# samuel-vitorino/sopro

Hardware: AMD Instinct MI355X
Metric: audio_seconds_per_second (higher is better)
Workload: dtype f32; 1 GPU; Sopro-135M synthesize, 32 utterances x 200 frames per GPU (BASELINE configs[1]), S=64 text tokens, 32 distinct 150-frame reference voice(s) per batch prepared outside the timed region, top_p=0.9 T=1.05 anti_loop (reference defaults), synthetic weights with EOS suppressed; batch_per_gpu=32, frames=200, voices_per_batch=32, parallelism=replicas x1 (utterance sharding, no collective), lanes_per_gpu=4

## Files before the change

sopro_amd/csrc/seanet_uptail.hip:

```cpp
#include <type_traits>
#include <utility>

#include "common.h"

namespace {

constexpr int FC = 128;
constexpr int FTI = 32;
constexpr int FTS = 4 * FTI;
constexpr int FXR = FTI + 1;
constexpr int FXROW = 2 * FC * 2 + 16;
constexpr int FHROW = 272;
constexpr int FHLD = FHROW / 4;
constexpr int FHR = FTS + 2;
constexpr int FYROW = 144;
constexpr int FW1B = 2 * 6 * 2;
constexpr int FW2B = 2 * 2 * 2;
constexpr int FCARRY = 2 * FHROW;
constexpr int FXBUF = FXR * FXROW;
constexpr int FUSE_LDS = 2 * FXBUF + 2 * FHR * FHROW + FTS * FYROW + (FW1B + FW2B) * 1024 + 2 * FCARRY;
static_assert(FUSE_LDS <= 160 * 1024, "LDS");
static_assert(FXBUF % 16 == 0 && (FHR * FHROW) % 16 == 0 && (FTS * FYROW) % 16 == 0, "16-byte aligned LDS regions");

typedef __bf16 fbf16x8 __attribute__((ext_vector_type(8)));
typedef float ff32x4 __attribute__((ext_vector_type(4)));
__device__ __forceinline__ fbf16x8 ffrag(const uint4& v) { return *reinterpret_cast<const fbf16x8*>(&v); }

__device__ __forceinline__ void fsplit8(const float* __restrict__ p, uint4& hi, uint4& lo) {
  const float4 a = *reinterpret_cast<const float4*>(p), b = *reinterpret_cast<const float4*>(p + 4);
  split2_bf16(a.x, a.y, hi.x, lo.x);
  split2_bf16(a.z, a.w, hi.y, lo.y);
  split2_bf16(b.x, b.y, hi.z, lo.z);
  split2_bf16(b.z, b.w, hi.w, lo.w);
}

__device__ __forceinline__ unsigned pair_rows(unsigned mine, unsigned sel) {
  const unsigned got = (unsigned)__builtin_amdgcn_update_dpp(0, (int)mine, 0xB1 , 0xF, 0xF, true);
  return __builtin_amdgcn_perm(got, mine, sel);
}

template <int... I, class F>
__device__ __forceinline__ void sfor_impl(std::integer_sequence<int, I...>, F&& f) {
  (f(std::integral_constant<int, I>()), ...);
}
template <int N, class F>
__device__ __forceinline__ void sfor(F&& f) {
  sfor_impl(std::make_integer_sequence<int, N>(), f);
}
template <int V>
using IC = std::integral_constant<int, V>;

template <int PASSES, bool XH>
__global__ __launch_bounds__(512, 1) void seanet_uptail_kernel(const void* __restrict__ x_, int64_t x_seg_stride, const float* __restrict__ wu,
                                                               const float* __restrict__ bu, const float* __restrict__ w1,
                                                               const float* __restrict__ b1, const float* __restrict__ w2,
                                                               const float* __restrict__ b2, const float* __restrict__ wf, float bf,
                                                               float* __restrict__ wav, int64_t wav_seg_stride, int T, int tiles) {
  static_assert(PASSES == 1 || PASSES == 3, "passes");
  static_assert(!XH || PASSES == 1, "bf16 rows are a one-pass (bf16 mode) input form");
  extern __shared__ __attribute__((aligned(16))) unsigned char lds[];
  unsigned char* xs = lds;
  unsigned char* hs = xs + 2 * FXBUF;
  unsigned char* hp = hs + FHR * FHROW;
  unsigned char* ys = hp + FHR * FHROW;
  uint4* w1s = reinterpret_cast<uint4*>(ys + FTS * FYROW);
  uint4* w2s = w1s + FW1B * 64;
  uint4* chs = w2s + FW2B * 64;
  uint4* cps = chs + FCARRY / 16;

  const int tid = threadIdx.x, lane = tid & 63, wave = tid >> 6;
  const int b = blockIdx.y;
  const int frow = lane & 31, fg = lane >> 5;
  const int col = lane & 15, kq = lane >> 4;
  const int ph = wave >> 1, cbase = 32 * (wave & 1);
  const bool odd = (lane & 1) != 0;
  const unsigned pair_sel = odd ? 0x03020706u : 0x05040100u;
  const int ntile = (T + FTI - 1) / FTI;
  const int tile0 = (int)blockIdx.x * tiles;
  if (tile0 >= ntile) return;
  const int kfirst = tile0 > 0 ? tile0 - 1 : 0;
  const int klast = min(tile0 + tiles, ntile) - 1;
  const int S = 4 * T;
  const float* xb = XH ? nullptr : reinterpret_cast<const float*>(x_) + (int64_t)b * x_seg_stride;
  const unsigned short* xb16 = XH ? reinterpret_cast<const unsigned short*>(x_) + (int64_t)b * x_seg_stride : nullptr;
  float* wb = wav + (int64_t)b * wav_seg_stride;

  constexpr int NV = XH ? 2 : 3;
  auto request = [&](int t0, int q) -> uint4 {
    const int idx = tid + q * 512;
    const int rr = XH ? idx >> 4 : idx >> 5, cc = XH ? idx & 15 : idx & 31;
    const int p = t0 + rr;
    const int pc = (rr < FXR && p <= T) ? p : 0;
    if constexpr (XH) return bulk_load16(xb16 + (int64_t)pc * FC + cc * 8, true);
    else return bulk_load16(xb + (int64_t)pc * FC + cc * 4, true);
  };
  auto stage = [&](unsigned char* xbuf, int q, const uint4& val) {
    const int idx = tid + q * 512;
    const int rr = XH ? idx >> 4 : idx >> 5, cc = XH ? idx & 15 : idx & 31;
    if (rr < FXR) {
      if constexpr (XH) {
        *reinterpret_cast<uint4*>(xbuf + rr * FXROW + cc * 16) = val;
      } else {
        uint2 hi, lo;
        split2_bf16(__uint_as_float(val.x), __uint_as_float(val.y), hi.x, lo.x);
        split2_bf16(__uint_as_float(val.z), __uint_as_float(val.w), hi.y, lo.y);
        *reinterpret_cast<uint2*>(xbuf + rr * FXROW + cc * 8) = hi;
        if (PASSES == 3) *reinterpret_cast<uint2*>(xbuf + rr * FXROW + 2 * FC + cc * 8) = lo;
      }
    }
  };
  {
    uint4 v0[NV], v1[NV];
#pragma unroll
    for (int q = 0; q < NV; ++q) v0[q] = request(kfirst * FTI, q);
#pragma unroll
    for (int q = 0; q < NV; ++q) v1[q] = request((kfirst + 1) * FTI, q);
#pragma unroll
    for (int q = 0; q < NV; ++q) stage(xs + (kfirst & 1) * FXBUF, q, v0[q]);
#pragma unroll
    for (int q = 0; q < NV; ++q) stage(xs + ((kfirst + 1) & 1) * FXBUF, q, v1[q]);
  }

  uint4 wh[16], wl[PASSES == 3 ? 16 : 1];
#pragma unroll
  for (int s = 0; s < 16; ++s) {
    uint4 lo;
    fsplit8(wu + (int64_t)(wave * 32 + frow) * (2 * FC) + s * 16 + fg * 8, wh[s], lo);
    if (PASSES == 3) wl[s] = lo;
    if ((s & 3) == 3) asm volatile("" ::: "memory");
  }
  const float bv = bu[wave * 32 + frow];
  for (int c = wave; c < 12; c += 8) {
    const int nt = c / 6, s = c % 6;
    uint4 hi, lo;
    fsplit8(w1 + (16 * nt + col) * 192 + s * 32 + kq * 8, hi, lo);
    w1s[((nt * 6 + s) * 2 + 0) * 64 + lane] = hi;
    w1s[((nt * 6 + s) * 2 + 1) * 64 + lane] = lo;
  }
  if (wave < 4) {
    const int half = wave >> 1, s = wave & 1;
    uint4 hi, lo;
    fsplit8(w2 + (half * 32 + frow) * 32 + s * 16 + fg * 8, hi, lo);
    w2s[((half * 2 + s) * 2 + 0) * 64 + lane] = hi;
    w2s[((half * 2 + s) * 2 + 1) * 64 + lane] = lo;
  }
  uint4 w1r[PASSES == 1 ? 2 : 1][PASSES == 1 ? 6 : 1];
  if (PASSES == 1) {
#pragma unroll
    for (int nt = 0; nt < 2; ++nt)
#pragma unroll
      for (int s = 0; s < 6; ++s) {
        uint4 lo;
        fsplit8(w1 + (16 * nt + col) * 192 + s * 32 + kq * 8, w1r[PASSES == 1 ? nt : 0][PASSES == 1 ? s : 0], lo);
      }
  }
  if (tid < 2 * FCARRY / 16) chs[tid] = make_uint4(0u, 0u, 0u, 0u);
  const float b1v[2] = {b1[col], b1[16 + col]};
  const float b2v = b2[cbase + frow];
  const float wl0 = wf[lane], wl1 = wf[64 + lane], wl2 = wf[128 + lane];

  f32x16 accP;
  float hraw[16];
#pragma unroll
  for (int q = 0; q < 16; ++q) accP[q] = 0.f;

  constexpr int NP = 16 * PASSES;
  uint4 pah, pal, nah, nal;
  pal = nal = make_uint4(0u, 0u, 0u, 0u);
  auto p_read = [&](const unsigned char* xt, int s) {
    const unsigned char* p = xt + frow * FXROW + fg * 16 + (s >> 3) * FXROW + (s & 7) * 32;
    nah = *reinterpret_cast<const uint4*>(p);
    if (PASSES == 3) nal = *reinterpret_cast<const uint4*>(p + 2 * FC);
  };
  auto p_mfma = [&](const unsigned char* xt, auto j_) {
    constexpr int J = decltype(j_)::value, s = J / PASSES, piece = J % PASSES;
    if constexpr (piece == 0) {
      pah = nah;
      if (PASSES == 3) pal = nal;
      if constexpr (s + 1 < 16) p_read(xt, s + 1);
    }
    if constexpr (PASSES == 3) {
      if constexpr (piece == 0) accP = __builtin_amdgcn_mfma_f32_32x32x16_bf16(ffrag(pal), ffrag(wh[s]), accP, 0, 0, 0);
      else if constexpr (piece == 1) accP = __builtin_amdgcn_mfma_f32_32x32x16_bf16(ffrag(pah), ffrag(wl[s]), accP, 0, 0, 0);
      else accP = __builtin_amdgcn_mfma_f32_32x32x16_bf16(ffrag(pah), ffrag(wh[s]), accP, 0, 0, 0);
    } else {
      accP = __builtin_amdgcn_mfma_f32_32x32x16_bf16(ffrag(pah), ffrag(wh[s]), accP, 0, 0, 0);
    }
  };
  auto p_slot = [&](const unsigned char* xt, auto j0_, auto j1_, auto i_, auto ns_) {
    constexpr int J0 = decltype(j0_)::value, J1 = decltype(j1_)::value, I = decltype(i_)::value, NS = decltype(ns_)::value;
    constexpr int lo = J0 + (J1 - J0) * I / NS, hi = J0 + (J1 - J0) * (I + 1) / NS;
    sfor<hi - lo>([&](auto d) { p_mfma(xt, IC<lo + decltype(d)::value>()); });
  };
  constexpr int JA = 10 * PASSES, JB = 12 * PASSES;

  auto h_raw = [&]() {
#pragma unroll
    for (int q = 0; q < 16; ++q) {
      hraw[q] = accP[q] + bv;
      accP[q] = 0.f;
    }
  };
  unsigned char* const hp0 = hs + (2 + ph + (odd ? 4 : 0)) * FHROW + (cbase + (frow & ~1)) * 2;
  auto h_elu = [&](auto i_) {
    constexpr int q = 2 * decltype(i_)::value;
    const int t = 8 * (q >> 2) + 4 * fg + (q & 3);
    unsigned hi, lo;
    split2_bf16(eluf_(hraw[q]), eluf_(hraw[q + 1]), hi, lo);
    unsigned char* hq = hp0 + 4 * t * FHROW;
    *reinterpret_cast<unsigned*>(hq) = pair_rows(hi, pair_sel);
    if (PASSES == 3) *reinterpret_cast<unsigned*>(hq + 128) = pair_rows(lo, pair_sel);
  };

  auto conv1 = [&](const unsigned char* xt) {
    ff32x4 acc[2] = {{0.f, 0.f, 0.f, 0.f}, {0.f, 0.f, 0.f, 0.f}};
    const unsigned char* a = hs + (16 * wave + col) * FHROW + kq * 16;
    sfor<6>([&](auto s_) {
      constexpr int s = decltype(s_)::value;
      {
        const unsigned char* p = a + (s >> 1) * FHROW + (s & 1) * 64;
        const uint4 ah = *reinterpret_cast<const uint4*>(p);
        if constexpr (PASSES == 3) {
          const uint4 al = *reinterpret_cast<const uint4*>(p + 128);
          const uint4 bh0 = w1s[((0 * 6 + s) * 2 + 0) * 64 + lane], bl0 = w1s[((0 * 6 + s) * 2 + 1) * 64 + lane];
          const uint4 bh1 = w1s[((1 * 6 + s) * 2 + 0) * 64 + lane], bl1 = w1s[((1 * 6 + s) * 2 + 1) * 64 + lane];
          p_slot(xt, IC<JA>(), IC<JB>(), s_, IC<10>());
          acc[0] = __builtin_amdgcn_mfma_f32_16x16x32_bf16(ffrag(al), ffrag(bh0), acc[0], 0, 0, 0);
          acc[1] = __builtin_amdgcn_mfma_f32_16x16x32_bf16(ffrag(al), ffrag(bh1), acc[1], 0, 0, 0);
          acc[0] = __builtin_amdgcn_mfma_f32_16x16x32_bf16(ffrag(ah), ffrag(bl0), acc[0], 0, 0, 0);
          acc[1] = __builtin_amdgcn_mfma_f32_16x16x32_bf16(ffrag(ah), ffrag(bl1), acc[1], 0, 0, 0);
          acc[0] = __builtin_amdgcn_mfma_f32_16x16x32_bf16(ffrag(ah), ffrag(bh0), acc[0], 0, 0, 0);
          acc[1] = __builtin_amdgcn_mfma_f32_16x16x32_bf16(ffrag(ah), ffrag(bh1), acc[1], 0, 0, 0);
        } else {
          p_slot(xt, IC<JA>(), IC<JB>(), s_, IC<10>());
          acc[0] = __builtin_amdgcn_mfma_f32_16x16x32_bf16(ffrag(ah), ffrag(w1r[0][PASSES == 1 ? s : 0]), acc[0], 0, 0, 0);
          acc[1] = __builtin_amdgcn_mfma_f32_16x16x32_bf16(ffrag(ah), ffrag(w1r[PASSES == 1 ? 1 : 0][PASSES == 1 ? s : 0]), acc[1], 0, 0, 0);
        }
      }
      __builtin_amdgcn_sched_barrier(0);
    });
    unsigned char* yp0 = ys + ((odd ? 32 : 0) + 4 * wave + kq) * FYROW + (col & ~1) * 2;
    sfor<4>([&](auto c_) {
      constexpr int c = decltype(c_)::value, nt = c >> 1, i = (c & 1) * 2;
      p_slot(xt, IC<JA>(), IC<JB>(), IC<6 + c>(), IC<10>());
      {
        unsigned hi, lo;
        split2_bf16(eluf_(acc[nt][i] + b1v[nt]), eluf_(acc[nt][i + 1] + b1v[nt]), hi, lo);
        unsigned char* yp = yp0 + i * 32 * FYROW + 32 * nt;
        *reinterpret_cast<unsigned*>(yp) = pair_rows(hi, pair_sel);
        if (PASSES == 3) *reinterpret_cast<unsigned*>(yp + 64) = pair_rows(lo, pair_sel);
      }
      __builtin_amdgcn_sched_barrier(0);
    });
  };

  constexpr int NC2 = 2 * PASSES;
  auto conv2 = [&](const unsigned char* xt) {
    f32x16 acc2;
#pragma unroll
    for (int q = 0; q < 16; ++q) acc2[q] = 0.f;
    const unsigned char* a = ys + (ph * 32 + frow) * FYROW + fg * 16;
    uint4 ah[2], al[2], bh[2], bl[2];
    {
#pragma unroll
      for (int s = 0; s < 2; ++s) {
        ah[s] = *reinterpret_cast<const uint4*>(a + s * 32);
        bh[s] = w2s[(((wave & 1) * 2 + s) * 2 + 0) * 64 + lane];
        if (PASSES == 3) {
          al[s] = *reinterpret_cast<const uint4*>(a + 64 + s * 32);
          bl[s] = w2s[(((wave & 1) * 2 + s) * 2 + 1) * 64 + lane];
        }
      }
    }
    sfor<NC2>([&](auto m_) {
      constexpr int m = decltype(m_)::value, s = m / PASSES, piece = m % PASSES;
      p_slot(xt, IC<JB>(), IC<NP>(), m_, IC<NC2 + 8>());
      {
        if constexpr (PASSES == 3) {
          if constexpr (piece == 0) acc2 = __builtin_amdgcn_mfma_f32_32x32x16_bf16(ffrag(al[s]), ffrag(bh[s]), acc2, 0, 0, 0);
          else if constexpr (piece == 1) acc2 = __builtin_amdgcn_mfma_f32_32x32x16_bf16(ffrag(ah[s]), ffrag(bl[s]), acc2, 0, 0, 0);
          else acc2 = __builtin_amdgcn_mfma_f32_32x32x16_bf16(ffrag(ah[s]), ffrag(bh[s]), acc2, 0, 0, 0);
        } else {
          acc2 = __builtin_amdgcn_mfma_f32_32x32x16_bf16(ffrag(ah[s]), ffrag(bh[s]), acc2, 0, 0, 0);
        }
      }
      __builtin_amdgcn_sched_barrier(0);
    });
    float* hf = reinterpret_cast<float*>(hp);
    sfor<8>([&](auto c_) {
      constexpr int q0 = 2 * decltype(c_)::value;
      p_slot(xt, IC<JB>(), IC<NP>(), IC<NC2 + decltype(c_)::value>(), IC<NC2 + 8>());
      {
#pragma unroll
        for (int q = q0; q < q0 + 2; ++q) {
          const int t = 8 * (q >> 2) + 4 * fg + (q & 3);
          hf[(2 + 4 * t + ph) * FHLD + cbase + frow] = eluf_(hraw[q] + acc2[q] + b2v);
        }
      }
      __builtin_amdgcn_sched_barrier(0);
    });
  };

  auto conv3 = [&](const unsigned char* xt, int s0, bool store, auto with_next_) {
    constexpr bool NEXT = decltype(with_next_)::value != 0;
    constexpr int NS3 = 8 + 8 + 8 + 4 + 2 + 1;
    const float* hf = reinterpret_cast<const float*>(hp);
    float xr[18], p16[16];
#pragma unroll
    for (int rr = 0; rr < 18; ++rr) xr[rr] = hf[(16 * wave + rr) * FHLD + lane];
    if constexpr (NEXT) {
      p_read(xt, 0);
      sfor<8>([&](auto c_) {
        p_slot(xt, IC<0>(), IC<JA>(), c_, IC<NS3>());
        h_elu(c_);
        __builtin_amdgcn_sched_barrier(0);
      });
    }
    sfor<8>([&](auto c_) {
      constexpr int i0 = 2 * decltype(c_)::value;
      if constexpr (NEXT) p_slot(xt, IC<0>(), IC<JA>(), IC<8 + decltype(c_)::value>(), IC<NS3>());
#pragma unroll
      for (int i = i0; i < i0 + 2; ++i) p16[i] = fmaf(wl2, xr[i + 2], fmaf(wl1, xr[i + 1], wl0 * xr[i]));
      __builtin_amdgcn_sched_barrier(0);
    });
    auto fu = [](float v) { return __float_as_uint(v); };
    sfor<8>([&](auto k_) {
      constexpr int k = decltype(k_)::value;
      if constexpr (NEXT) p_slot(xt, IC<0>(), IC<JA>(), IC<16 + k>(), IC<NS3>());
      const auto r = __builtin_amdgcn_permlane32_swap(fu(p16[k]), fu(p16[k + 8]), false, false);
      p16[k] = __uint_as_float(r[0]) + __uint_as_float(r[1]);
      __builtin_amdgcn_sched_barrier(0);
    });
    sfor<4>([&](auto k_) {
      constexpr int k = decltype(k_)::value;
      if constexpr (NEXT) p_slot(xt, IC<0>(), IC<JA>(), IC<24 + k>(), IC<NS3>());
      const auto r = __builtin_amdgcn_permlane16_swap(fu(p16[k]), fu(p16[k + 4]), false, false);
      p16[k] = __uint_as_float(r[0]) + __uint_as_float(r[1]);
      __builtin_amdgcn_sched_barrier(0);
    });
    {
      const bool up8 = (lane & 8) != 0, up4 = (lane & 4) != 0;
      sfor<2>([&](auto k_) {
        constexpr int k = decltype(k_)::value;
        if constexpr (NEXT) p_slot(xt, IC<0>(), IC<JA>(), IC<28 + k>(), IC<NS3>());
        const float keep = up8 ? p16[k + 2] : p16[k], send = up8 ? p16[k] : p16[k + 2];
        p16[k] = keep + __uint_as_float((unsigned)__builtin_amdgcn_update_dpp(0, (int)fu(send), 0x128 , 0xF, 0xF, true));
        __builtin_amdgcn_sched_barrier(0);
      });
      if constexpr (NEXT) p_slot(xt, IC<0>(), IC<JA>(), IC<30>(), IC<NS3>());
      const float keep = up4 ? p16[1] : p16[0], send = up4 ? p16[0] : p16[1];
      int got = __builtin_amdgcn_update_dpp(0, (int)fu(send), 0x114 , 0xF, 0xA, false);
      got = __builtin_amdgcn_update_dpp(got, (int)fu(send), 0x104 , 0xF, 0x5, false);
      p16[0] = keep + __uint_as_float((unsigned)got);
    }
    float sum = p16[0];
    sum += __uint_as_float((unsigned)__builtin_amdgcn_update_dpp(0, (int)fu(sum), 0xB1 , 0xF, 0xF, true));
    sum += __uint_as_float((unsigned)__builtin_amdgcn_update_dpp(0, (int)fu(sum), 0x4E , 0xF, 0xF, true));
    const int sidx = s0 + 16 * wave + (lane >> 2);
    if ((lane & 3) == 0 && store && sidx < S) wb[sidx] = sum + bf;
  };

  __syncthreads();
  {
    const unsigned char* x0 = xs + (kfirst & 1) * FXBUF;
    p_read(x0, 0);
    sfor<NP>([&](auto j_) { p_mfma(x0, j_); });
    h_raw();
    sfor<8>([&](auto c_) { h_elu(c_); });
    if (wave == 0 && lane < FCARRY / 16) reinterpret_cast<uint4*>(hs)[lane] = chs[lane];
    const unsigned char* x1 = xs + ((kfirst + 1) & 1) * FXBUF;
    p_read(x1, 0);
    sfor<JA>([&](auto j_) { p_mfma(x1, j_); });
  }
  uint4 vq = request((kfirst + 2) * FTI, 0);
  __syncthreads();

  for (int k = kfirst; k <= klast; ++k) {
    const bool nxt = k < klast;
    const bool store = k >= tile0;
    const unsigned char* x1 = xs + ((k + 1) & 1) * FXBUF;
    unsigned char* x2 = xs + (k & 1) * FXBUF;
    const int t2 = (k + 2) * FTI;
    stage(x2, 0, vq);
    vq = request(t2, 1);
    uint4 vq2 = make_uint4(0u, 0u, 0u, 0u);
    if (NV == 3) vq2 = request(t2, 2);
    conv1(x1);
    if (wave == 7 && lane < FCARRY / 16) chs[lane] = reinterpret_cast<const uint4*>(hs + FTS * FHROW)[lane];
    __syncthreads();
    stage(x2, 1, vq);
    if (NV == 3) stage(x2, 2, vq2);
    conv2(x1);
    if (wave == 5 && lane < FCARRY / 16) reinterpret_cast<uint4*>(hp)[lane] = cps[lane];
    __syncthreads();
    if (nxt) {
      vq = request((k + 3) * FTI, 0);
      h_raw();
      conv3(x2, k * FTS, store, IC<1>());
      if (wave == 0 && lane < FCARRY / 16) reinterpret_cast<uint4*>(hs)[lane] = chs[lane];
    } else {
      conv3(x2, k * FTS, store, IC<0>());
    }
    if (wave == 6 && lane < FCARRY / 16) cps[lane] = reinterpret_cast<const uint4*>(hp + FTS * FHROW)[lane];
    if (!nxt) break;
    __syncthreads();
  }
}

int g_uptail_tiles = 0;

template <int PASSES, bool XH>
int launch_uptail(const void* x, int64_t x_seg_stride, const float* wu, const float* bu, const float* w1, const float* b1, const float* w2,
                  const float* b2, const float* wf, float bf, float* wav, int64_t wav_seg_stride, int32_t B, int32_t T, hipStream_t s) {
  const int ntile = (T + FTI - 1) / FTI;
  int tiles = g_uptail_tiles ? g_uptail_tiles : (int)(((int64_t)ntile * B + 2047) / 2048);
  if (!g_uptail_tiles && tiles < 24) tiles = ntile < 24 ? ntile : 24;
  if (tiles < 1) tiles = 1;
  auto kern = seanet_uptail_kernel<PASSES, XH>;
  SOPRO_SET_MAX_LDS_ONCE(kern, FUSE_LDS);
  hipLaunchKernelGGL(kern, dim3((unsigned)((ntile + tiles - 1) / tiles), (unsigned)B), dim3(512), FUSE_LDS, s, x, x_seg_stride, wu, bu, w1, b1, w2, b2, wf,
                     bf, wav, wav_seg_stride, T, tiles);
  SOPRO_LAUNCH_CHECK();
}

}

extern "C" int sopro_seanet_uptail_set_tiles(int tiles) {
  g_uptail_tiles = tiles > 0 ? tiles : 0;
  return 0;
}

extern "C" int sopro_seanet_uptail_f32(const float* x, int64_t x_seg_stride, const float* wu, const float* bu, const float* w1, const float* b1,
                                       const float* w2, const float* b2, const float* wf, float bf, float* wav, int64_t wav_seg_stride, int32_t B,
                                       int32_t T, int32_t passes, void* stream) {
  SOPRO_CHECK_ARG(x && wu && bu && w1 && b1 && w2 && b2 && wf && wav && B > 0 && T > 0, "bad pointers or sizes");
  SOPRO_CHECK_ARG(passes == 1 || passes == 3, "passes must be 3 (three-pass split-bf16) or 1 (bf16 mode)");
  SOPRO_CHECK_ARG(aligned16(x) && aligned16(wu) && aligned16(w1) && aligned16(w2) && (x_seg_stride & 3) == 0, "x, wu, w1, w2 16-byte aligned, x segment stride % 4 == 0");
  SOPRO_CHECK_ARG(B == 1 || (x_seg_stride >= (int64_t)(T + 1) * FC && wav_seg_stride >= (int64_t)4 * T),
                  "segment strides: x holds T + 1 rows of 128 per utterance (one zero row in front), wav 4 T samples");
  if (passes == 3) return launch_uptail<3, false>(x, x_seg_stride, wu, bu, w1, b1, w2, b2, wf, bf, wav, wav_seg_stride, B, T, (hipStream_t)stream);
  return launch_uptail<1, false>(x, x_seg_stride, wu, bu, w1, b1, w2, b2, wf, bf, wav, wav_seg_stride, B, T, (hipStream_t)stream);
}

extern "C" int sopro_seanet_uptail_bf16(const void* x, int64_t x_seg_stride, const float* wu, const float* bu, const float* w1, const float* b1,
                                        const float* w2, const float* b2, const float* wf, float bf, float* wav, int64_t wav_seg_stride, int32_t B,
                                        int32_t T, void* stream) {
  SOPRO_CHECK_ARG(x && wu && bu && w1 && b1 && w2 && b2 && wf && wav && B > 0 && T > 0, "bad pointers or sizes");
  SOPRO_CHECK_ARG(aligned16(x) && aligned16(wu) && aligned16(w1) && aligned16(w2) && (x_seg_stride & 7) == 0, "x, wu, w1, w2 16-byte aligned, x segment stride % 8 == 0");
  SOPRO_CHECK_ARG(B == 1 || (x_seg_stride >= (int64_t)(T + 1) * FC && wav_seg_stride >= (int64_t)4 * T),
                  "segment strides: x holds T + 1 rows of 128 per utterance (one zero row in front), wav 4 T samples");
  return launch_uptail<1, true>(x, x_seg_stride, wu, bu, w1, b1, w2, b2, wf, bf, wav, wav_seg_stride, B, T, (hipStream_t)stream);
}
```

Measured before the change: 27490 audio-s/s.

## Split and swizzle hidden and conv1-output LDS buffers to avoid bank conflicts

Replaces the padded interleaved row layouts of the upsampled hidden buffer and the conv1 output buffer with separate 64-byte and 32-byte row planes for each channel half and hi/lo bf16 part. Rows are permuted and 16-byte chunks XOR-swizzled, with the writer and reader address maps changed to match. The aim is to remove LDS bank conflicts on the MFMA operand loads and the paired-row stores in conv1 and conv2. The carry copy between tiles is rewritten for the new layout, which brings more complex address arithmetic and a risk of indexing mistakes.

```diff
diff --git a/sopro_amd/csrc/seanet_uptail.hip b/sopro_amd/csrc/seanet_uptail.hip
--- a/sopro_amd/csrc/seanet_uptail.hip
+++ b/sopro_amd/csrc/seanet_uptail.hip
@@ -10,17 +10,23 @@
 constexpr int FTS = 4 * FTI;
 constexpr int FXR = FTI + 1;
 constexpr int FXROW = 2 * FC * 2 + 16;
+constexpr int FHSROW = 64;
+constexpr int FHSPL = 132 * FHSROW;
+constexpr int FHSLO = 2 * FHSPL;
 constexpr int FHROW = 272;
 constexpr int FHLD = FHROW / 4;
 constexpr int FHR = FTS + 2;
-constexpr int FYROW = 144;
+constexpr int FYROW = 32;
+constexpr int FYNT = FTS * FYROW;
+constexpr int FYLO = 2 * FYNT;
 constexpr int FW1B = 2 * 6 * 2;
 constexpr int FW2B = 2 * 2 * 2;
-constexpr int FCARRY = 2 * FHROW;
+constexpr int FCARRYH = 8 * FHSROW;
+constexpr int FCARRYP = 2 * FHROW;
 constexpr int FXBUF = FXR * FXROW;
-constexpr int FUSE_LDS = 2 * FXBUF + 2 * FHR * FHROW + FTS * FYROW + (FW1B + FW2B) * 1024 + 2 * FCARRY;
+constexpr int FUSE_LDS = 2 * FXBUF + 4 * FHSPL + FHR * FHROW + 4 * FYNT + (FW1B + FW2B) * 1024 + FCARRYH + FCARRYP;
 static_assert(FUSE_LDS <= 160 * 1024, "LDS");
-static_assert(FXBUF % 16 == 0 && (FHR * FHROW) % 16 == 0 && (FTS * FYROW) % 16 == 0, "16-byte aligned LDS regions");
+static_assert(FXBUF % 16 == 0 && FHSPL % 256 == 0 && (FHR * FHROW) % 16 == 0 && FYNT % 256 == 0, "16-byte aligned LDS regions");
 
 typedef __bf16 fbf16x8 __attribute__((ext_vector_type(8)));
 typedef float ff32x4 __attribute__((ext_vector_type(4)));
@@ -33,6 +39,11 @@
   split2_bf16(b.x, b.y, hi.z, lo.z);
   split2_bf16(b.z, b.w, hi.w, lo.w);
 }
+
+__device__ __forceinline__ int hrowp(int row) { return (row & ~7) | ((row >> 2) & 1) | ((row & 3) << 1); }
+__device__ __forceinline__ int hswz(int row) { return row & 2; }
+__device__ __forceinline__ int yrow(int row) { return (row & 0x45) | ((((row >> 5) ^ (row >> 1)) & 1) << 1) | ((row & 2) << 2) | ((row & 8) << 1) | ((row & 16) << 1); }
+__device__ __forceinline__ int yswz(int row) { return (row >> 3) & 1; }
 
 __device__ __forceinline__ unsigned pair_rows(unsigned mine, unsigned sel) {
   const unsigned got = (unsigned)__builtin_amdgcn_update_dpp(0, (int)mine, 0xB1 , 0xF, 0xF, true);
@@ -61,12 +72,12 @@
   extern __shared__ __attribute__((aligned(16))) unsigned char lds[];
   unsigned char* xs = lds;
   unsigned char* hs = xs + 2 * FXBUF;
-  unsigned char* hp = hs + FHR * FHROW;
+  unsigned char* hp = hs + 4 * FHSPL;
   unsigned char* ys = hp + FHR * FHROW;
-  uint4* w1s = reinterpret_cast<uint4*>(ys + FTS * FYROW);
+  uint4* w1s = reinterpret_cast<uint4*>(ys + 4 * FYNT);
   uint4* w2s = w1s + FW1B * 64;
   uint4* chs = w2s + FW2B * 64;
-  uint4* cps = chs + FCARRY / 16;
+  uint4* cps = chs + FCARRYH / 16;
 
   const int tid = threadIdx.x, lane = tid & 63, wave = tid >> 6;
   const int b = blockIdx.y;
@@ -154,7 +165,7 @@
         fsplit8(w1 + (16 * nt + col) * 192 + s * 32 + kq * 8, w1r[PASSES == 1 ? nt : 0][PASSES == 1 ? s : 0], lo);
       }
   }
-  if (tid < 2 * FCARRY / 16) chs[tid] = make_uint4(0u, 0u, 0u, 0u);
+  if (tid < (FCARRYH + FCARRYP) / 16) chs[tid] = make_uint4(0u, 0u, 0u, 0u);
   const float b1v[2] = {b1[col], b1[16 + col]};
   const float b2v = b2[cbase + frow];
   const float wl0 = wf[lane], wl1 = wf[64 + lane], wl2 = wf[128 + lane];
@@ -201,27 +212,33 @@
       accP[q] = 0.f;
     }
   };
-  unsigned char* const hp0 = hs + (2 + ph + (odd ? 4 : 0)) * FHROW + (cbase + (frow & ~1)) * 2;
+  const int hrow0 = 2 + ph + (odd ? 4 : 0);
+  const bool hcopy = (lane & 4) == 0;
+  auto hcarry = [&](int row) { return reinterpret_cast<uint4*>(hs + (lane >> 4) * FHSPL + (row + 2 * ((lane >> 3) & 1)) * FHSROW) + (lane & 3); };
+  uint4* const hside = chs + ((lane & 3) | ((lane >> 3) << 2));
+  unsigned char* const hp0 = hs + (wave & 1) * FHSPL + hrowp(hrow0) * FHSROW + 16 * ((frow >> 3) ^ hswz(hrow0)) + (frow & 6) * 2;
   auto h_elu = [&](auto i_) {
     constexpr int q = 2 * decltype(i_)::value;
     const int t = 8 * (q >> 2) + 4 * fg + (q & 3);
     unsigned hi, lo;
     split2_bf16(eluf_(hraw[q]), eluf_(hraw[q + 1]), hi, lo);
-    unsigned char* hq = hp0 + 4 * t * FHROW;
+    unsigned char* hq = hp0 + 4 * t * FHSROW;
     *reinterpret_cast<unsigned*>(hq) = pair_rows(hi, pair_sel);
-    if (PASSES == 3) *reinterpret_cast<unsigned*>(hq + 128) = pair_rows(lo, pair_sel);
+    if (PASSES == 3) *reinterpret_cast<unsigned*>(hq + FHSLO) = pair_rows(lo, pair_sel);
   };
 
   auto conv1 = [&](const unsigned char* xt) {
     ff32x4 acc[2] = {{0.f, 0.f, 0.f, 0.f}, {0.f, 0.f, 0.f, 0.f}};
-    const unsigned char* a = hs + (16 * wave + col) * FHROW + kq * 16;
+    const unsigned char* a[3];
+#pragma unroll
+    for (int tap = 0; tap < 3; ++tap) a[tap] = hs + hrowp(16 * wave + col + tap) * FHSROW + 16 * (kq ^ hswz(16 * wave + col + tap));
     sfor<6>([&](auto s_) {
       constexpr int s = decltype(s_)::value;
       {
-        const unsigned char* p = a + (s >> 1) * FHROW + (s & 1) * 64;
+        const unsigned char* p = a[s >> 1] + (s & 1) * FHSPL;
         const uint4 ah = *reinterpret_cast<const uint4*>(p);
         if constexpr (PASSES == 3) {
-          const uint4 al = *reinterpret_cast<const uint4*>(p + 128);
+          const uint4 al = *reinterpret_cast<const uint4*>(p + FHSLO);
           const uint4 bh0 = w1s[((0 * 6 + s) * 2 + 0) * 64 + lane], bl0 = w1s[((0 * 6 + s) * 2 + 1) * 64 + lane];
           const uint4 bh1 = w1s[((1 * 6 + s) * 2 + 0) * 64 + lane], bl1 = w1s[((1 * 6 + s) * 2 + 1) * 64 + lane];
           p_slot(xt, IC<JA>(), IC<JB>(), s_, IC<10>());
@@ -239,16 +256,17 @@
       }
       __builtin_amdgcn_sched_barrier(0);
     });
-    unsigned char* yp0 = ys + ((odd ? 32 : 0) + 4 * wave + kq) * FYROW + (col & ~1) * 2;
+    const int yrow0 = (odd ? 32 : 0) + 4 * wave + kq;
+    unsigned char* yp0 = ys + yrow(yrow0) * FYROW + 16 * ((col >> 3) ^ yswz(yrow0)) + (col & 6) * 2;
     sfor<4>([&](auto c_) {
       constexpr int c = decltype(c_)::value, nt = c >> 1, i = (c & 1) * 2;
       p_slot(xt, IC<JA>(), IC<JB>(), IC<6 + c>(), IC<10>());
       {
         unsigned hi, lo;
         split2_bf16(eluf_(acc[nt][i] + b1v[nt]), eluf_(acc[nt][i + 1] + b1v[nt]), hi, lo);
-        unsigned char* yp = yp0 + i * 32 * FYROW + 32 * nt;
+        unsigned char* yp = yp0 + i * 32 * FYROW + nt * FYNT;
         *reinterpret_cast<unsigned*>(yp) = pair_rows(hi, pair_sel);
-        if (PASSES == 3) *reinterpret_cast<unsigned*>(yp + 64) = pair_rows(lo, pair_sel);
+        if (PASSES == 3) *reinterpret_cast<unsigned*>(yp + FYLO) = pair_rows(lo, pair_sel);
       }
       __builtin_amdgcn_sched_barrier(0);
     });
@@ -259,15 +277,15 @@
     f32x16 acc2;
 #pragma unroll
     for (int q = 0; q < 16; ++q) acc2[q] = 0.f;
-    const unsigned char* a = ys + (ph * 32 + frow) * FYROW + fg * 16;
+    const unsigned char* a = ys + yrow(ph * 32 + frow) * FYROW + 16 * (fg ^ yswz(ph * 32 + frow));
     uint4 ah[2], al[2], bh[2], bl[2];
     {
 #pragma unroll
       for (int s = 0; s < 2; ++s) {
-        ah[s] = *reinterpret_cast<const uint4*>(a + s * 32);
+        ah[s] = *reinterpret_cast<const uint4*>(a + s * FYNT);
         bh[s] = w2s[(((wave & 1) * 2 + s) * 2 + 0) * 64 + lane];
         if (PASSES == 3) {
-          al[s] = *reinterpret_cast<const uint4*>(a + 64 + s * 32);
+          al[s] = *reinterpret_cast<const uint4*>(a + FYLO + s * FYNT);
           bl[s] = w2s[(((wave & 1) * 2 + s) * 2 + 1) * 64 + lane];
         }
       }
@@ -367,7 +385,7 @@
     sfor<NP>([&](auto j_) { p_mfma(x0, j_); });
     h_raw();
     sfor<8>([&](auto c_) { h_elu(c_); });
-    if (wave == 0 && lane < FCARRY / 16) reinterpret_cast<uint4*>(hs)[lane] = chs[lane];
+    if (wave == 0 && hcopy) *hcarry(0) = *hside;
     const unsigned char* x1 = xs + ((kfirst + 1) & 1) * FXBUF;
     p_read(x1, 0);
     sfor<JA>([&](auto j_) { p_mfma(x1, j_); });
@@ -386,22 +404,22 @@
     uint4 vq2 = make_uint4(0u, 0u, 0u, 0u);
     if (NV == 3) vq2 = request(t2, 2);
     conv1(x1);
-    if (wave == 7 && lane < FCARRY / 16) chs[lane] = reinterpret_cast<const uint4*>(hs + FTS * FHROW)[lane];
+    if (wave == 7 && hcopy) *hside = *hcarry(FTS);
     __syncthreads();
     stage(x2, 1, vq);
     if (NV == 3) stage(x2, 2, vq2);
     conv2(x1);
-    if (wave == 5 && lane < FCARRY / 16) reinterpret_cast<uint4*>(hp)[lane] = cps[lane];
+    if (wave == 5 && lane < FCARRYP / 16) reinterpret_cast<uint4*>(hp)[lane] = cps[lane];
     __syncthreads();
     if (nxt) {
       vq = request((k + 3) * FTI, 0);
       h_raw();
       conv3(x2, k * FTS, store, IC<1>());
-      if (wave == 0 && lane < FCARRY / 16) reinterpret_cast<uint4*>(hs)[lane] = chs[lane];
+      if (wave == 0 && hcopy) *hcarry(0) = *hside;
     } else {
       conv3(x2, k * FTS, store, IC<0>());
     }
-    if (wave == 6 && lane < FCARRY / 16) cps[lane] = reinterpret_cast<const uint4*>(hp + FTS * FHROW)[lane];
+    if (wave == 6 && lane < FCARRYP / 16) cps[lane] = reinterpret_cast<const uint4*>(hp + FTS * FHROW)[lane];
     if (!nxt) break;
     __syncthreads();
   }
```

Result: no change. 27350 audio-s/s (-0.5%).
